# swyoon/Diffusion-by-MaxEntIRL

Hardware: AMD Instinct MI355X
Metric: images/sec (CIFAR-10 DDPM T=10 generation) (higher is better)
Workload: dtype bf16; 1 GPU; CIFAR-10 DDPM U-Net (35.7M params) VARSampler T=10 generation, 256 images/GPU/step, 3x32x32 (BASELINE configs[1]); noise drawn inside the step; global_batch=256, T=10, parallelism=dp1 (independent trajectories, no collective)

## Files before the change

### diffusion-by-maxentirl_amd/csrc/conv_igemm.hip

```cpp
#include "conv_common.h"

namespace {

template <int MB, int NB, int CK, int PMAX>
__global__ __launch_bounds__(256) void conv_igemm_kernel(ConvArgs p) {
    constexpr int WAVES_PX = 8 / NB;
    constexpr int WAVES_CO = 4 / WAVES_PX;
    constexpr int BN = 32 * MB * WAVES_CO;
    constexpr int ROWB = CK * 2 + 16;
    constexpr int KSTEPS = CK / 16;
    constexpr int PPP = CK / 8;
    extern __shared__ __attribute__((aligned(16))) char smem[];

    const int tid = threadIdx.x;
    const int lane = tid & 63;
    const int wave = __builtin_amdgcn_readfirstlane(tid >> 6);
    const int wco = wave % WAVES_CO;
    const int wpx = wave / WAVES_CO;

    int pt, cot;
    if (!conv_block_to_tile(p, blockIdx.x, pt, cot)) return;

    const bool k27 = p.in_mode == DXMI_IN_NCHW_F32_K27;
    const bool rows = p.in_mode == DXMI_IN_ROWS_F32;
// ... 383 lines not shown
    const int HP = flat ? 256 : a.SUBS * a.HH * a.HWd;
    p->lds = (size_t)HP * (CK * 2 + 16);
    b.lds_buf = (int)p->lds;
    const int npieces = HP * (CK / 8);
    const int pmax = npieces <= 6 * 256 ? 6 : (npieces <= 9 * 256 ? 9 : 0);
    const bool wide = a.Cout % 128 == 0 && a.out_mode != DXMI_OUT_NCHW_F32;
    b.CT = wide ? a.Cout / 128 : a.CB;
    p->kind = ConvKernel::igemm;
    p->t0 = wide && variant == 1 ? 2 : 1;
    p->t1 = !wide ? 2 : (variant == 1 ? 4 : 8);
    p->t2 = pmax;
    p->grid = (a.PT + 7) / 8 * 8 * b.CT;
    p->id = p->t0 * 1000 + p->t1 * 100 + pmax;
}

template <int MB, int NB>
int launch_igemm(const ConvPlan& p, hipStream_t st) {
    return p.t2 == 6 ? launch_conv<MB, NB, 32, 6>(p.args, p.lds, st)
                     : p.t2 == 9 ? launch_conv<MB, NB, 32, 9>(p.args, p.lds, st) : launch_conv<MB, NB, 32, 0>(p.args, p.lds, st);
}

void conv_select(const ConvArgs& a, int variant, ConvPlan* p) {
    auto is = [&](bool (*select)(const ConvArgs&, ConvPlan*)) { *p = ConvPlan{}; p->args = a; return select(a, p); };
    if (variant == 0 && (a.gn_out ? is(conv_sm_select) || is(conv_ws8_select)
                                  : is(conv_ws_select) || is(conv1x1_rw8_select) || is(conv1x1_rw_select) || is(conv_head_select) ||
                                        is(conv_sm_select) || is(conv_ws8_select) || is(conv_stem_select) || is(conv_pipe_select)))
        return;
    *p = ConvPlan{};
    p->args = a;
    conv_igemm_select(a, variant, p);
}

int conv_launch(const ConvPlan& p, hipStream_t st) {
    switch (p.kind) {
    case ConvKernel::ws: return conv_ws_launch(p, st);
    case ConvKernel::ws8: return conv_ws8_launch(p, st);
    case ConvKernel::sm: return conv_sm_launch(p, st);
    case ConvKernel::rw: return conv1x1_rw_launch(p, st);
    case ConvKernel::rw8: return conv1x1_rw8_launch(p, st);
    case ConvKernel::head: return conv_head_launch(p, st);
    case ConvKernel::stem: return conv_stem_launch(p, st);
    case ConvKernel::pipe:
    case ConvKernel::stream1x1: return conv_pipe_launch(p, st);
    case ConvKernel::igemm: break;
    }
    if (p.t0 == 2) return launch_igemm<2, 4>(p, st);
    return p.t1 == 8 ? launch_igemm<1, 8>(p, st) : launch_igemm<1, 2>(p, st);
// ... 205 lines not shown
```

### diffusion-by-maxentirl_amd/csrc/conv_ws.hip

```cpp
#include "conv_common.h"
#include <stdlib.h>
#include <type_traits>


#ifdef DXMI_CONV_STAMPS
__device__ unsigned g_ws_wait[256][176];
extern "C" int dxmi_debug_read_ws_stamps(void* dst, int bytes) {
    return (int)hipMemcpyFromSymbol(dst, HIP_SYMBOL(g_ws_wait), bytes, 0, hipMemcpyDeviceToHost);
}
#define WS_STAMPED_BARRIER(idx)                                                                     \
    do {                                                                                            \
        const unsigned long long t0_ = __builtin_amdgcn_s_memtime();                                \
        ws_barrier();                                                                               \
        const unsigned long long t1_ = __builtin_amdgcn_s_memtime();                                \
        if (wave == 0 && lane == 0 && (idx) < 160 && blockIdx.x < 256) g_ws_wait[blockIdx.x][(idx)] = (unsigned)(t1_ - t0_); \
    } while (0)
#define WS_CLOCKSTAMP(slot, cond)                                                                    \
    do {                                                                                            \
        if ((cond) && lane == 0 && blockIdx.x < 256) {                                              \
            g_ws_wait[blockIdx.x][(slot)] = (unsigned)__builtin_amdgcn_s_memtime();                 \
            g_ws_wait[blockIdx.x][(slot) + 1] = (unsigned)__builtin_amdgcn_s_memrealtime();         \
        }                                                                                           \
    } while (0)
#define WS_TSTAMP(slot, cond)                                                                        \
// ... 3 lines not shown
#define WS_DBG(bit) (p.stagger & (bit))
#else
#define WS_STAMPED_BARRIER(idx) ws_barrier()
#define WS_TSTAMP(slot, cond) do {} while (0)
#define WS_CLOCKSTAMP(slot, cond) do {} while (0)
#define WS_DBG(bit) 0
#endif

__device__ unsigned long long g_ws_clock[4];
extern "C" int dxmi_conv_ws_last_clock(unsigned long long* host_out4) {
    return hipMemcpyFromSymbol(host_out4, HIP_SYMBOL(g_ws_clock), 4 * sizeof(unsigned long long), 0, hipMemcpyDeviceToHost) == hipSuccess ? DXMI_OK
                                                                                                                                          : DXMI_ELAUNCH;
}

namespace {

constexpr int WS_A_SLOT = 8192;
constexpr int WS_RING = 6;
constexpr int WS_A_RING = WS_RING * WS_A_SLOT;
constexpr int WS_RO = 256 * 256;
constexpr int WS_TB = 1024;
constexpr int WS_HALO_BLOCKS = 22;
constexpr int WS_HALO = WS_HALO_BLOCKS * 1024;

__device__ uint4 ws_zero16 = {0u, 0u, 0u, 0u};

#define WS_GPTR(p) ((const __attribute__((address_space(1))) void*)(p))
#define WS_LPTR(p) ((__attribute__((address_space(3))) void*)(p))

__device__ __forceinline__ void ws_barrier() { asm volatile("s_waitcnt lgkmcnt(0)\n\ts_barrier" ::: "memory"); }

#define WS_INTERLEAVE_4()                                       \
    do {                                                        \
        _Pragma("unroll") for (int i_ = 0; i_ < 4; ++i_) {      \
            __builtin_amdgcn_sched_group_barrier(0x008, 3, 0);  \
            __builtin_amdgcn_sched_group_barrier(0x100, 1, 0);  \
        }                                                       \
        __builtin_amdgcn_sched_group_barrier(0x008, 4, 0);      \
    } while (0)
#define WS_INTERLEAVE_8()                                       \
    do {                                                        \
        _Pragma("unroll") for (int i_ = 0; i_ < 8; ++i_) {      \
            __builtin_amdgcn_sched_group_barrier(0x008, 1, 0);  \
            __builtin_amdgcn_sched_group_barrier(0x100, 1, 0);  \
        }                                                       \
        __builtin_amdgcn_sched_group_barrier(0x008, 8, 0);      \
// ... 43 lines not shown
                ws_f32x2 x = {__builtin_bit_cast(float, raw[i] << 16), __builtin_bit_cast(float, raw[i] & 0xffff0000u)};
                ws_f32x2 y = x * A[i] + B[i];
                const ws_f32x2 t = y * ws_f32x2{-1.4426950408889634f, -1.4426950408889634f};
                ws_f32x2 e = {__builtin_amdgcn_exp2f(t[0]), __builtin_amdgcn_exp2f(t[1])};
                e = e + ws_f32x2{1.f, 1.f};
                const ws_f32x2 rc = {__builtin_amdgcn_rcpf(e[0]), __builtin_amdgcn_rcpf(e[1])};
                y = y * rc;
                bf16x2 o = {(bf16)y[0], (bf16)y[1]};
                sink ^= __builtin_bit_cast(unsigned, o);
            }
            raw += u32x4{0x10001u, 0x20003u, 0x10002u, 0x30001u};
        }
    }
};
#define WS_VALU_DECL(lane_) WsValuLoad vl_; vl_.init(lane_)
#define WS_VALU_RUN() vl_.run()
#define WS_VALU_DONE() do { if (vl_.sink == 0x12345u) reinterpret_cast<volatile unsigned*>(p.out)[0] = vl_.sink; } while (0)
#else
#define WS_VALU_DECL(lane_) do {} while (0)
#define WS_VALU_RUN() do {} while (0)
#define WS_VALU_DONE() do {} while (0)
#endif

template <int TW>
__device__ __forceinline__ void conv_ws_body(const ConvArgs& p) {
    constexpr int TH = 256 / TW, HP = TW == 32 ? 34 : 18, HH = TH + 2, TWl = TW == 32 ? 5 : 4;
    extern __shared__ __attribute__((aligned(1024))) char smem[];
    char* const halo0 = smem;
    char* const aring = smem + 2 * WS_HALO;
    char* const ro = aring + WS_A_RING;
    float* const tb = reinterpret_cast<float*>(ro + WS_RO);

    const int tid = threadIdx.x, lane = tid & 63;
    const int wave = __builtin_amdgcn_readfirstlane(tid >> 6);
    const int txn = p.OW / TW, tyn = p.OH / TH;
    const int nchunks = (p.C0 + p.C1) / 32;
    const int S = 9 * nchunks;
    const int ntiles = p.PT * p.CT;
    const int ups = p.ups ? 1 : 0;

    auto tile_of = [&](int q, WsTile& t) {
        t.cot = q % p.CT;
        const int pt = q / p.CT;
        const int tx = pt % txn, ty = (pt / txn) % tyn;
        t.n0 = pt / (txn * tyn);
        t.oy0 = ty * TH;
        t.ox0 = tx * TW;
    };

    const int q0 = dxmi_xcd_logical(blockIdx.x, gridDim.x, p.xcd_order);
    int q = q0;
    if (q >= ntiles) return;
    const int qstride = gridDim.x;
    if (blockIdx.x == 0 && tid == 0) {
// ... 51 lines not shown
        (void)stamp_i;
        for (;;) {
            const bool more = q + qstride < ntiles;
            for (int c = 0; c < nchunks; c += 2) {
#pragma unroll
                for (int u = 0; u < 18; ++u) {
                    read_b(u, 1, By);
                    if (u & 1) mfma16(A1, Bx, 0); else mfma16(A0, Bx, 0);
                    WS_INTERLEAVE_4();
                    if (u % 3 == 2) { if (!(WS_DBG(16))) WS_STAMPED_BARRIER(stamp_i + c * 9 + u); }
                    if (u & 1) read_a(u + 1, A0); else read_a(u + 1, A1);
                    read_b(u + 1, 0, Bx);
                    if (u & 1) mfma16(A1, By, 1); else mfma16(A0, By, 1);
                    WS_INTERLEAVE_8();
                    __builtin_amdgcn_sched_barrier(0);
                }
            }
            WS_TSTAMP(158, wave == 0 && q == q0);
            ws_barrier();
            WS_TSTAMP(159, wave == 0 && q == q0);
            {
                const bool plain = p.act == DXMI_ACT_NONE;
                char* const rowb = ro + ((ph * 128 + px) << 8) + 8 * (kg & 1);
                const bool want_stats = p.gn_stats != nullptr;
                const int cot_ = q % p.CT;
                float* const stp = want_stats ? p.gn_stats + ((size_t)((q / p.CT) * 2 + ph) * (p.Cout >> 1) + cot_ * 64 + ch * 32 + kg * 2) * 2 : nullptr;
                auto epi = [&](auto RES, auto MASK, auto ACT, auto STATS) {
                    constexpr bool kRes = decltype(RES)::value, kMask = decltype(MASK)::value, kAct = decltype(ACT)::value, kStats = decltype(STATS)::value;
#pragma unroll
                    for (int cb = 0; cb < 4; ++cb) {
                        float st[4] = {0.f, 0.f, 0.f, 0.f};
                        const int co = ch * 64 + cb * 16 + 4 * kg;
                        const f32x4 b0 = *reinterpret_cast<const f32x4*>(tb + co), t0 = *reinterpret_cast<const f32x4*>(tb + 128 + co);
                        f32x4 bv;
#pragma unroll
                        for (int e = 0; e < 4; ++e) bv[e] = b0[e] + t0[e];
                        char* const a0 = rowb + (((ch * 8 + cb * 2 + (kg >> 1)) ^ px) << 4);
                        bf16x4 r[8];
                        if constexpr (kRes) {
#pragma unroll
                            for (int nb = 0; nb < 8; ++nb) r[nb] = *reinterpret_cast<const bf16x4*>(a0 + nb * 4096);
                        }
#pragma unroll
                        for (int nb = 0; nb < 8; ++nb) {
                            f32x4 v;
#pragma unroll
                            for (int e = 0; e < 4; ++e) v[e] = acc[cb][nb][e] + bv[e];
                            if constexpr (kRes) {
                                if constexpr (kMask) {
#pragma unroll
                                    for (int e = 0; e < 4; ++e) v[e] *= ((float)r[nb][e] > 0.f ? 1.f : p.mask_slope);
                                } else {
#pragma unroll
                                    for (int e = 0; e < 4; ++e) v[e] += (float)r[nb][e];
                                }
                            }
                            if constexpr (kAct) {
#pragma unroll
                                for (int e = 0; e < 4; ++e) v[e] = dxmi_act_lin(v[e], slope);
                            }
                            bf16x4 o;
#pragma unroll
                            for (int e = 0; e < 4; ++e) o[e] = (bf16)v[e];
                            *reinterpret_cast<bf16x4*>(a0 + nb * 4096) = o;
                            if constexpr (kStats) dxmi_stats4(o, st);
#pragma unroll
                            for (int e = 0; e < 4; ++e) acc[cb][nb][e] = 0.f;
                        }
                        if constexpr (kStats) {
#pragma unroll
                            for (int e = 0; e < 4; ++e) st[e] = dxmi_row16_sum(st[e]);
                            if (px == 0 && cot_ * 128 + co < p.Cout) {
                                f32x4 sv;
#pragma unroll
                                for (int e = 0; e < 4; ++e) sv[e] = st[e];
                                *reinterpret_cast<f32x4*>(stp + cb * 16) = sv;
                            }
                        }
                    }
                };
                using T_ = std::true_type;
                using F_ = std::false_type;
                const bool is_mask = has_res && p.res_is_mask;
                if (plain && !is_mask) {
                    if (has_res) { if (want_stats) epi(T_{}, F_{}, F_{}, T_{}); else epi(T_{}, F_{}, F_{}, F_{}); }
                    else { if (want_stats) epi(F_{}, F_{}, F_{}, T_{}); else epi(F_{}, F_{}, F_{}, F_{}); }
                } else if (!want_stats) {
                    if (is_mask) { if (plain) epi(T_{}, T_{}, F_{}, F_{}); else epi(T_{}, T_{}, T_{}, F_{}); }
                    else if (has_res) epi(T_{}, F_{}, T_{}, F_{});
                    else epi(F_{}, F_{}, T_{}, F_{});
                } else {
                    if (is_mask) epi(T_{}, T_{}, T_{}, T_{});
                    else if (has_res) epi(T_{}, F_{}, T_{}, T_{});
                    else epi(F_{}, F_{}, T_{}, T_{});
                }
            }
            WS_TSTAMP(166, wave == 0 && q == q0);
            ws_barrier();
            WS_TSTAMP(157, wave == 0 && q == q0);
            if (!more) {
                WS_CLOCKSTAMP(170, wave == 0);
                break;
            }
            q += qstride;
            stamp_i += S;
        }
    } else if (wave < 6) {
        WS_VALU_DECL(lane);
        const int lw = wave - 4;
        const char* const wb = reinterpret_cast<const char*>(p.w) + (size_t)lane * 16;
        WsTile cur;
        tile_of(q, cur);
        auto issue_tap = [&](int cot, int g) {
            if (WS_DBG(1)) return;
            const int c = g / 9, t = g - c * 9;
            char* dst = aring + (g % WS_RING) * WS_A_SLOT + lw * 4096;
            const char* src = wb + ((size_t)(t * p.KST + c * 2 + lw) * p.CB) * 1024;
#pragma unroll
            for (int f = 0; f < 4; ++f) {
                const int cb = cot * 4 + f < p.CB ? cot * 4 + f : p.CB - 1;
// ... 35 lines not shown
        bool first_tile_l = true, first_group0 = true;
        load_group(0, cur.cot, cur.cot, fq[0]);
        load_group(1, cur.cot, cur.cot, fq[1]);
        asm volatile("s_waitcnt vmcnt(12)" ::: "memory");
        store_group(0, fq[0]);
        asm volatile("s_waitcnt lgkmcnt(0)" ::: "memory");
        load_group(2, cur.cot, cur.cot, fq[0]);
        ws_barrier();
        bool first_tile = true;
        for (;;) {
            const bool more = q + qstride < ntiles;
            WsTile nxt = cur;
            if (more) tile_of(q + qstride, nxt);
            if (!first_tile && lw == 0 && !(WS_DBG(8))) {
                const int co_a = cur.cot * 128 + lane, co_b = co_a + 64 < p.Cout ? co_a + 64 : p.Cout - 1;
                if (p.bias) {
                    __builtin_amdgcn_global_load_lds(WS_GPTR(p.bias + co_a), WS_LPTR(tb), 4, 0, 0);
                    __builtin_amdgcn_global_load_lds(WS_GPTR(p.bias + co_b), WS_LPTR(tb + 64), 4, 0, 0);
                }
                if (p.addvec) {
                    const float* av = p.addvec + (size_t)cur.n0 * p.addvec_ld;
                    __builtin_amdgcn_global_load_lds(WS_GPTR(av + co_a), WS_LPTR(tb + 128), 4, 0, 0);
                    __builtin_amdgcn_global_load_lds(WS_GPTR(av + co_b), WS_LPTR(tb + 192), 4, 0, 0);
                }
            }
            const bf16* const res_t = p.residual + ((((size_t)cur.n0 * p.OH + cur.oy0) * p.OW + cur.ox0) * p.Cout + cur.cot * 128);
            const bool res_here = !first_tile_l && p.residual != nullptr && !(WS_DBG(8));
            first_tile_l = false;
            first_tile = false;
            for (int G0 = 0; G0 < NG; G0 += 2) {
#pragma unroll
                for (int j = 0; j < 2; ++j) {
                    const int G = G0 + j;
                    if (G > 0 || first_group0) {
                        asm volatile("s_waitcnt vmcnt(12)" ::: "memory");
                        store_group(G + 1, fq[(j + 1) & 1]);
                        asm volatile("s_waitcnt lgkmcnt(0)" ::: "memory");
                    }
                    if (res_here && G > 0) {
                        const int cg = (G - 1) / 3, g3 = (G - 1) - cg * 3;
                        if (cg + 1 < nchunks) {
                            const int k0 = cg * kpc_l < 32 ? cg * kpc_l : 32, k1 = k0 + kpc_l < 32 ? k0 + kpc_l : 32;
                            const int i0 = g3 < 2 ? 3 * g3 : 6, i1 = g3 < 2 ? 3 * g3 + 3 : 12;
                            const int ka = k0 + i0 < k1 ? k0 + i0 : k1, kb = k0 + i1 < k1 ? k0 + i1 : k1;
#pragma unroll 1
                            for (int k = ka; k < kb; ++k) {
                                const int rel = ((k >> (TWl - 3)) * p.OW + (k & (TW / 8 - 1)) * 8) * p.Cout + ((k & 1) ? lpar_l1 : lpar_l0);
                                const bool ok = cur.cot * 128 + ((k & 1) ? c8o_l : c8e_l) * 8 < p.Cout;
                                const void* g = ok ? (const void*)(res_t + rel) : (const void*)zero_page_l;
                                __builtin_amdgcn_global_load_lds(WS_GPTR(g), WS_LPTR(ro + (k * 128 + lw * 64) * 16), 16, 0, 0);
                            }
                        }
                    }
                    if (G > 0 || first_group0) load_group(G + 3, cur.cot, more ? nxt.cot : cur.cot, fq[(j + 1) & 1]);
                    WS_TSTAMP(151, wave == 4 && G == 0 && q == q0 + qstride);
                    WS_VALU_RUN();
                    if (!(WS_DBG(16))) ws_barrier();
                }
            }
            first_group0 = false;
            if (more) {
                asm volatile("s_waitcnt vmcnt(12)" ::: "memory");
                store_group(1, fq[1]);
                asm volatile("s_waitcnt lgkmcnt(0)" ::: "memory");
                load_group(3, nxt.cot, nxt.cot, fq[1]);
            }
            ws_barrier();
            ws_barrier();
            WS_TSTAMP(150, wave == 4 && q == q0);
            if (!more) break;
            q += qstride;
            cur = nxt;
        }
        asm volatile("s_waitcnt vmcnt(0)" ::: "memory");
        WS_VALU_DONE();
    } else if (wave == 6) {
        WS_VALU_DECL(lane);
        constexpr int HBA = WS_HALO_BLOCKS;
        const char* const zero_page = reinterpret_cast<const char*>(p.mask_src);
        int hrel0[HBA], hrel1[HBA];
        unsigned m_in = 0, m_top = 0, m_bot = 0, m_left = 0, m_right = 0;
#pragma unroll
        for (int k = 0; k < HBA; ++k) {
            const int hp = k * 16 + (lane >> 2);
            const int hy = hp / HP, hx = hp - hy * HP;
            const int rel = ((hy - 1) >> ups) * p.IW + ((hx - 1) >> ups);
            const int j8 = ((lane & 3) ^ (2 * ((hx >> 2) & 1))) * 8;
            hrel0[k] = (rel * p.C0 + j8) * 2;
            hrel1[k] = (rel * p.C1 + j8) * 2;
            m_in |= (unsigned)(hy < HH && hx < TW + 2) << k;
// ... 23 lines not shown
            for (int k = 0; k < HBA; ++k) {
                if (k < ka || k >= kb) continue;
                const char* g = (hmask >> k) & 1 ? base + (first ? hrel0[k] : hrel1[k]) : zero_page;
                __builtin_amdgcn_global_load_lds(WS_GPTR(g), WS_LPTR(buf + k * 1024), 16, 0, 0);
            }
        };
        WsTile cur;
        tile_of(q, cur);
        if (!p.bias) { tb[lane] = 0.f; tb[64 + lane] = 0.f; }
        if (!p.addvec) { tb[128 + lane] = 0.f; tb[192 + lane] = 0.f; }
        halo_plan(cur);
        halo_issue(0, halo0, 0, HBA);
        if (!(WS_DBG(8))) {
            const int co_a = cur.cot * 128 + lane, co_b = co_a + 64 < p.Cout ? co_a + 64 : p.Cout - 1;
            if (p.bias) {
                __builtin_amdgcn_global_load_lds(WS_GPTR(p.bias + co_a), WS_LPTR(tb), 4, 0, 0);
                __builtin_amdgcn_global_load_lds(WS_GPTR(p.bias + co_b), WS_LPTR(tb + 64), 4, 0, 0);
            }
            if (p.addvec) {
                const float* av = p.addvec + (size_t)cur.n0 * p.addvec_ld;
                __builtin_amdgcn_global_load_lds(WS_GPTR(av + co_a), WS_LPTR(tb + 128), 4, 0, 0);
                __builtin_amdgcn_global_load_lds(WS_GPTR(av + co_b), WS_LPTR(tb + 192), 4, 0, 0);
            }
        }
        asm volatile("s_waitcnt vmcnt(0)" ::: "memory");
        ws_barrier();
        WsTile nxt = cur;
        for (;;) {
            const bool more = q + qstride < ntiles;
            for (int c = 0; c < nchunks; ++c) {
                const bool wrap = c + 1 == nchunks;
                if (wrap && more) {
                    tile_of(q + qstride, nxt);
                    halo_plan(nxt);
                }
                const bool do_halo = !wrap || more;
                char* const hbuf = halo0 + ((c + 1) & 1) * WS_HALO;
                const int hc = wrap ? 0 : c + 1;
#pragma unroll
                for (int t = 0; t < 9; ++t) {
                    if (t < 8 && do_halo) halo_issue(hc, hbuf, 3 * t, 3 * t + 3 < HBA ? 3 * t + 3 : HBA);
                    if (t == 8) asm volatile("s_waitcnt vmcnt(0)" ::: "memory");
                    if (t % 3 == 2) { WS_VALU_RUN(); if (!(WS_DBG(16))) ws_barrier(); }
                }
            }
            ws_barrier();
            ws_barrier();
            if (!more) break;
            q += qstride;
            cur = nxt;
        }
        WS_VALU_DONE();
    } else if (wave == 7) {
        WS_VALU_DECL(lane);
        const char* const zero_page = reinterpret_cast<const char*>(p.mask_src);
        const int prA = lane >> 4, prB = 4 + (lane >> 4), lc = lane & 15;
        const int lparA[2] = {prA * p.Cout + ((lc ^ prA) * 8), prA * p.Cout + ((lc ^ (prA | 8)) * 8)};
        const int lparB[2] = {prB * p.Cout + ((lc ^ prB) * 8), prB * p.Cout + ((lc ^ (prB | 8)) * 8)};
        const int c8A[2] = {lc ^ prA, lc ^ (prA | 8)}, c8B[2] = {lc ^ prB, lc ^ (prB | 8)};
        auto tile_base = [&](const WsTile& t) -> size_t {
            return (((size_t)t.n0 * p.OH + t.oy0) * p.OW + t.ox0) * p.Cout + t.cot * 128;
        };
        auto piece_u = [&](int k) -> int { return ((k >> (TWl - 3)) * p.OW + (k & (TW / 8 - 1)) * 8) * p.Cout; };
        WsTile cur;
        tile_of(q, cur);
        if (p.residual != nullptr && !(WS_DBG(8))) {
            const bf16* rb = p.residual + tile_base(cur);
#pragma unroll 1
            for (int k = 0; k < 32; ++k) {
// ... 29 lines not shown
                    piece_range(c, t, ka, kb);
                    if (ka < kb && do_drain) {
                        bf16x8 va[2], vb[2];
#pragma unroll
                        for (int u = 0; u < 2; ++u)
                            if (ka + u < kb) {
                                va[u] = *reinterpret_cast<const bf16x8*>(ro + ((ka + u) * 128 + lane) * 16);
                                vb[u] = *reinterpret_cast<const bf16x8*>(ro + ((ka + u) * 128 + 64 + lane) * 16);
                            }
#pragma unroll
                        for (int u = 0; u < 2; ++u)
                            if (ka + u < kb) {
                                const int k = ka + u, pu = piece_u(k);
                                if (prev.cot * 128 + c8A[k & 1] * 8 < p.Cout) *reinterpret_cast<bf16x8*>(out_prev + pu + lparA[k & 1]) = va[u];
                                if (prev.cot * 128 + c8B[k & 1] * 8 < p.Cout) *reinterpret_cast<bf16x8*>(out_prev + pu + lparB[k & 1]) = vb[u];
                            }
                    }
                    asm volatile("s_waitcnt lgkmcnt(0)" ::: "memory");
                    if (t % 3 == 2) { WS_VALU_RUN(); if (!(WS_DBG(16))) ws_barrier(); }
                }
            }
            if (!have_prev) asm volatile("s_waitcnt vmcnt(0)" ::: "memory");
            ws_barrier();
            ws_barrier();
            out_prev = reinterpret_cast<bf16*>(p.out) + tile_base(cur);
            prev = cur;
            have_prev = true;
            if (!more) break;
            q += qstride;
            cur = nxt;
        }
        WS_VALU_DONE();
    }

    {
        const int qlast = q0 + ((ntiles - 1 - q0) / qstride) * qstride;
        WsTile lt;
        tile_of(qlast, lt);
        bf16* const ob = reinterpret_cast<bf16*>(p.out) + ((((size_t)lt.n0 * p.OH + lt.oy0) * p.OW + lt.ox0) * p.Cout + lt.cot * 128);
        const int t2 = tid & 127, kq = tid >> 7;
        const int pr = t2 >> 4;
#pragma unroll
        for (int i = 0; i < 8; i += 4) {
            bf16x8 v[4];
#pragma unroll
            for (int u = 0; u < 4; ++u) v[u] = *reinterpret_cast<const bf16x8*>(ro + (((i + u) * 4 + kq) * 128 + t2) * 16);
#pragma unroll
            for (int u = 0; u < 4; ++u) {
                const int k = (i + u) * 4 + kq;
                const int lp = k * 8 + pr;
                const int c8 = (t2 & 15) ^ (lp & 15);
                const int rel = ((lp >> TWl) * p.OW + (lp & (TW - 1))) * p.Cout + c8 * 8;
                if (lt.cot * 128 + c8 * 8 < p.Cout) *reinterpret_cast<bf16x8*>(ob + rel) = v[u];
            }
        }
        WS_CLOCKSTAMP(174, wave == 0);
    }
    if (blockIdx.x == 0 && tid == 0) {
        g_ws_clock[2] = __builtin_amdgcn_s_memtime();
        g_ws_clock[3] = __builtin_amdgcn_s_memrealtime();
    }
}

template <int TW>
__global__ __launch_bounds__(512, 1) void conv_ws_kernel(ConvArgs p) {
    conv_ws_body<TW>(p);
}

}

bool conv_ws_select(const ConvArgs& a, ConvPlan* p) {
    if (a.in_mode != DXMI_IN_NHWC_BF16 || a.out_mode != DXMI_OUT_NHWC_BF16) return false;
    if (a.ksize != 3 || a.stride != 1 || a.pad != 1 || a.ups == 2 || (a.mask_src && a.residual) || a.act == DXMI_ACT_SILU) return false;
    if (a.Cout % 64 != 0 || (a.C0 + a.C1) % 32 != 0 || a.C0 % 32 != 0) return false;
    const int TW = a.OW >= 32 ? 32 : a.OW;
    if (TW != 32 && TW != 16) return false;
    const int TH = 256 / TW;
    if (a.OH % TH != 0 || a.OW % TW != 0) return false;
    const int nchunks = (a.C0 + a.C1) / 32;
    if ((9 * nchunks) % WS_RING != 0 || nchunks % 2 != 0) return false;
    if (nchunks < 4) return false;
    const int min_tiles = dxmi_tuning("conv_ws_min_tiles");
    if ((long)a.N * (a.OH / TH) * (a.OW / TW) * ((a.Cout + 127) / 128) < min_tiles) return false;
    if ((long)a.N * a.IH * a.IW * (a.C0 > a.C1 ? a.C0 : a.C1) * 2 >= (1L << 31)) return false;
    ConvArgs& b = p->args;
    if (a.mask_src) { b.residual = a.mask_src; b.res_is_mask = 1; }
    b.SUBS = 1;
    b.PT = a.N * (a.OH / TH) * (a.OW / TW);
    b.CT = (a.Cout + 127) / 128;
    b.tile_px = 256;
    b.xcd_order = 1;
    b.stagger = 0;
    p->kind = ConvKernel::ws; p->t0 = TW;
    p->grid = b.PT * b.CT < 256 ? b.PT * b.CT : 256;
    p->lds = 2 * WS_HALO + WS_A_RING + WS_RO + WS_TB;
    p->id = 400000 + TW;
    p->stats_tile = 128;
    conv_ws_up_select(a, p);
    return true;
}

int conv_ws_launch(const ConvPlan& p, hipStream_t st) {
    if (p.t1 == 1) return conv_ws_up_launch(p, st);
    static const void* zero_page = nullptr;
    DXMI_CHECK_ARG(conv_zero_page(zero_page, HIP_SYMBOL(ws_zero16)), "dxmi_conv2d_fwd(ws): hipGetSymbolAddress(ws_zero16) failed");
    ConvArgs b = p.args;
    b.mask_src = reinterpret_cast<const bf16*>(zero_page);
#ifdef DXMI_CONV_STAMPS
    static const int dbg = getenv("DXMI_CONV_WS_DBG") ? atoi(getenv("DXMI_CONV_WS_DBG")) : 0;
    b.stagger = dbg;
#endif
    static bool attr_set = false;
    if (!attr_set) {
        (void)hipFuncSetAttribute(reinterpret_cast<const void*>(conv_ws_kernel<32>), hipFuncAttributeMaxDynamicSharedMemorySize, 160 * 1024);
        (void)hipFuncSetAttribute(reinterpret_cast<const void*>(conv_ws_kernel<16>), hipFuncAttributeMaxDynamicSharedMemorySize, 160 * 1024);
        attr_set = true;
    }
    if (p.t0 == 32) hipLaunchKernelGGL(conv_ws_kernel<32>, dim3(p.grid), dim3(512), p.lds, st, b);
    else hipLaunchKernelGGL(conv_ws_kernel<16>, dim3(p.grid), dim3(512), p.lds, st, b);
    DXMI_CHECK_LAUNCH("dxmi_conv2d_fwd(ws)");
    return DXMI_OK;
}
```

### diffusion-by-maxentirl_amd/dxmi_hip/ops.py

```python
import ctypes
import math
import os

import torch

from . import _lib
from . import graph as _graph
from ._lib import ConvDesc, check, load

ACT_NONE, ACT_LEAKY02, ACT_RELU, ACT_SILU = 0, 1, 2, 3
IN_NHWC_BF16, IN_NCHW_F32_K27 = 0, 1
OUT_NHWC_BF16, OUT_NCHW_F32 = 0, 1


_RAW_STREAM = getattr(torch._C, "_cuda_getCurrentRawStream", None)
_GET_DEVICE = getattr(torch._C, "_cuda_getDevice", None)


def _stream():
    if _RAW_STREAM is not None and _GET_DEVICE is not None:
        return ctypes.c_void_p(_RAW_STREAM(_GET_DEVICE()))
    return ctypes.c_void_p(torch.cuda.current_stream().cuda_stream)


# ... 156 lines not shown

def pack_conv_weight(w, transpose_flip=False, k27=False, out=None):
    _need_cuda(w)
    if w.dim() == 2:
        w = w[:, :, None, None]
    w = w.detach().contiguous().float()
    O, I, k, _ = w.shape
    Cout, Cin = (I, O) if transpose_flip else (O, I)
    lib = load()
    nbytes = lib.dxmi_packed_conv_weight_bytes(Cout, Cin, k, int(k27))
    if out is None:
        out = pack_tensor(nbytes, torch.uint8, w.device)
    assert out.numel() == nbytes
    if _PACK_BATCH is not None:
        _PACK_BATCH.append((w, out, Cout, Cin, k, transpose_flip, k27))
    else:
        check(lib.dxmi_pack_conv_weight(_ptr(w), _ptr(out), Cout, Cin, k, int(transpose_flip), int(k27), _stream()),
              "dxmi_pack_conv_weight")
    return PackedConvWeight(out, Cout, Cin, k, k27, transpose_flip)


class BlockStats:

    __slots__ = ("buf", "P")

    def __init__(self, buf, P):
        self.buf, self.P = buf, P


_STATS_P = {}


def conv2d(x, pw, *, in1=None, bias=None, addvec=None, residual=None, stride=1, pad=None, pad_br=None, upsample=False,
           act=ACT_NONE, out=None, out_nchw_f32=False, variant=0, mask_src=None, mask_slope=0.0, want_stats=False, fuse_gn=None):
    _need_cuda(x, in1, bias, addvec, residual, out)
    k = pw.ksize
    if pad is None:
        pad = k // 2
    d = ConvDesc()
    if pw.k27:
        N, _, IH, IW = x.shape
        C0, C1 = 3, 0
        assert x.dtype == torch.float32 and x.is_contiguous()
    else:
        N, IH, IW, C0 = x.shape
        C1 = in1.shape[3] if in1 is not None else 0
        assert x.dtype == torch.bfloat16 and x.is_contiguous()
        assert in1 is None or (in1.dtype == torch.bfloat16 and in1.is_contiguous() and in1.shape[:3] == x.shape[:3])
        assert C0 + C1 == pw.Cin, f"conv2d: input channels {C0}+{C1} != packed Cin {pw.Cin}"
    VIH, VIW = (IH * 2, IW * 2) if upsample else (IH, IW)
    if pad_br is None:
        pad_br = pad
    OH, OW = (VIH + pad + pad_br - k) // stride + 1, (VIW + pad + pad_br - k) // stride + 1
    Cout = pw.Cout
    if out is None:
        if out_nchw_f32:
            out = torch.empty((N, Cout, OH, OW), dtype=torch.float32, device=x.device)
# ... 11 lines not shown
        assert residual.dtype == torch.bfloat16 and residual.is_contiguous() and tuple(residual.shape) == (N, OH, OW, Cout)
    d.residual = residual.data_ptr() if residual is not None else None
    d.out = out.data_ptr()
    d.N, d.IH, d.IW, d.C0, d.C1, d.OH, d.OW, d.Cout = N, IH, IW, C0, C1, OH, OW, Cout
    d.ksize, d.stride, d.pad, d.upsample, d.act = k, stride, pad, int(upsample), act
    d.in_mode = IN_NCHW_F32_K27 if pw.k27 else IN_NHWC_BF16
    d.out_mode = OUT_NCHW_F32 if out_nchw_f32 else OUT_NHWC_BF16
    d.variant = variant
    if mask_src is not None:
        assert mask_src.dtype == torch.bfloat16 and mask_src.is_contiguous() and tuple(mask_src.shape) == (N, OH, OW, Cout)
    d.mask_src = mask_src.data_ptr() if mask_src is not None else None
    d.mask_slope = float(mask_slope)
    d.gn_stats = None
    stats = None
    if want_stats and not out_nchw_f32 and variant == 0:
        key = (N, IH, IW, C0, C1, OH, OW, Cout, k, stride, pad, int(upsample), act, d.in_mode, residual is not None, mask_src is not None)
        P = _STATS_P.get(key)
        if P is None:
            P = _STATS_P[key] = int(load().dxmi_conv2d_gn_stats_partials(ctypes.byref(d)))
        if P > 0:
            stats = BlockStats(torch.empty((N, P, Cout // 2, 2), dtype=torch.float32, device=x.device), P)
            d.gn_stats = stats.buf.data_ptr()
    d.gn_out, y = None, None
    if fuse_gn is not None:
        assert not want_stats
        gamma, beta, groups, eps, silu, keep_raw = fuse_gn
        d.gn_groups = groups
        d.gn_flags = int(bool(silu)) | (0 if keep_raw else 2)
        key = ("gn", N, IH, IW, C0, C1, OH, OW, Cout, k, stride, pad, int(upsample), act, d.in_mode, d.out_mode, variant,
               residual is not None, mask_src is not None, groups, bool(keep_raw))
        ok = _STATS_P.get(key)
        if ok is None:
            ok = _STATS_P[key] = int(load().dxmi_conv2d_gn_fuse_supported(ctypes.byref(d)))
        if ok:
            assert gamma.dtype == torch.float32 and beta.dtype == torch.float32 and gamma.numel() == Cout and beta.numel() == Cout
            y = torch.empty((N, OH, OW, Cout), dtype=torch.bfloat16, device=x.device)
            d.gn_out, d.gn_gamma, d.gn_beta, d.gn_eps = y.data_ptr(), gamma.data_ptr(), beta.data_ptr(), float(eps)
    if PROFILER is not None:
        PROFILER.launch_conv(d)
    else:
        check(load().dxmi_conv2d_fwd(ctypes.byref(d), _stream()), "dxmi_conv2d_fwd")
    if fuse_gn is not None:
        return (out if (y is None or fuse_gn[5]) else None), y
    if stats is not None and stats.P > MAX_APPLY_PARTIALS:
        stats = fold_stats(stats)
    return (out, stats) if want_stats else out


class OpProfiler:

    def __init__(self):
        self.records = []

    def bracket(self, cls, name, flops, nbytes, fn):
        e0, e1 = torch.cuda.Event(enable_timing=True), torch.cuda.Event(enable_timing=True)
        e0.record()
        out = fn()
        e1.record()
        self.records.append((cls, name, float(flops), float(nbytes), e0, e1))
        return out

    def launch_conv(self, d):
        lib = load()
        kid = lib.dxmi_conv2d_kernel_id(ctypes.byref(d))
        cin = 27 if d.in_mode == IN_NCHW_F32_K27 else (d.C0 + d.C1) * d.ksize * d.ksize
        flops = 2.0 * d.N * d.OH * d.OW * d.Cout * cin
        in_b = d.N * d.IH * d.IW * (d.C0 + d.C1) * (4 if d.in_mode == IN_NCHW_F32_K27 else 2)
        out_b = d.N * d.OH * d.OW * d.Cout * (4 if d.out_mode == OUT_NCHW_F32 else 2)
        res_b = out_b if d.residual else 0
        if d.gn_out:
            res_b += out_b if not (d.gn_flags & 2) else 0
        w_b = d.Cout * cin * 2
        cls = "conv_other" if kid >= 600000 else "conv1x1" if kid >= 500000 else "conv3x3" if kid >= 400000 else "conv_stem" if kid >= 300000 else ("conv1x1" if kid >= 200000 else ("conv3x3" if kid >= 30000 else "conv_other"))
        if kid == 400008 and d.gn_out:
            kid = 400009
        self.bracket(cls, kid, flops, in_b + out_b + res_b + w_b,
                     lambda: check(lib.dxmi_conv2d_fwd(ctypes.byref(d), _stream()), "dxmi_conv2d_fwd"))

    def summary(self):
        out = {}
        for cls, name, fl, by, e0, e1 in self.records:
            s = out.setdefault((cls, name), {"launches": 0, "ms": 0.0, "flops": 0.0, "bytes": 0.0})
            s["launches"] += 1
            s["ms"] += e0.elapsed_time(e1)
            s["flops"] += fl
            s["bytes"] += by
        return out


PROFILER = None


def _prof(cls, name, flops, nbytes, fn):
    return fn() if PROFILER is None else PROFILER.bracket(cls, name, flops, nbytes, fn)


_WS = {}

# ... 1804 lines not shown
```

### diffusion-by-maxentirl_amd/models/DxMI/unet_small.py

```python
import os

import torch
import torch.nn as nn

from dxmi_hip import ops
from dxmi_hip._lib import DxmiError
from dxmi_hip.packs import PackedWeights, WeightPacks


def Normalize(in_channels):
    return nn.GroupNorm(num_groups=32, num_channels=in_channels, eps=1e-6, affine=True)


def _conv(cin, cout, k, stride=1, padding=0):
    return nn.Conv2d(cin, cout, kernel_size=k, stride=stride, padding=padding)


class Upsample(nn.Module):

    def __init__(self, in_channels, with_conv):
        super().__init__()
        self.with_conv = with_conv
        if with_conv:
            self.conv = _conv(in_channels, in_channels, 3, 1, 1)
# ... 142 lines not shown
            ps.pack((id(b), "conv2"), b.conv2.weight)
            if b.in_channels != b.out_channels:
                sc = b.conv_shortcut if b.use_conv_shortcut else b.nin_shortcut
                ps.pack((id(b), "short"), sc.weight)
        for m in self.modules():
            if isinstance(m, AttnBlock):
                ps.pack((id(m), "qkv"), ps.stage_cat([m.q.weight, m.k.weight, m.v.weight]))
                pk[id(m), "qkv_bias"] = ps.stage_cat([m.q.bias, m.k.bias, m.v.bias])
                ps.pack((id(m), "proj"), m.proj_out.weight)
                if m.in_channels == 256:
                    ps.derived((id(m), "proj_attn"), lambda out, m=m: ops.pack_attn_proj_weight(m.proj_out.weight, out=out))
                    ps.derived((id(m), "block"), lambda out, m=m: ops.attn_block_pack(
                        m.q.weight, m.q.bias, m.k.weight, m.v.weight, m.v.bias, m.proj_out.weight, m.proj_out.bias,
                        float(int(m.in_channels) ** (-0.5)), out=out))
            elif isinstance(m, (Upsample, Downsample)):
                ps.pack((id(m), "conv"), m.conv.weight)
        ps.pack("conv_in", self.conv_in.weight, k27=(self.in_channels == 3))
        ps.pack("conv_out", self.conv_out.weight)

    FUSE_ATTN_PROJ = True
    FUSE_GN_SHORTCUT = os.environ.get("DXMI_GN_SHORTCUT", "1") != "0"
    FUSE_ATTN_BLOCK = True
    FUSE_GN_SMALL = True
    STREAM_GN_MIN_HW = 256

    def _conv_s(self, x, pw, **kw):
        out, st = ops.conv2d(x, pw, want_stats=True, **kw)
        if st is None and out.shape[1] * out.shape[2] >= self.STREAM_GN_MIN_HW:
            st = ops.block_stats(out)
        return out, st

    def _resblock(self, pk, b, x0, x1, tp, s0=None, s1=None, nxt=None):
        stream = x0.shape[1] * x0.shape[2] >= self.STREAM_GN_MIN_HW
        fused = None
        if isinstance(s0, _Normed):
            assert s0.norm is b.norm1 and x1 is None
            a0 = s0.y
        else:
            if self.FUSE_GN_SHORTCUT and stream and b.in_channels != b.out_channels and not b.use_conv_shortcut:
                fused = ops.groupnorm_silu_shortcut(x0, b.norm1.weight, b.norm1.bias, pk[id(b), "short"], in1=x1, bias=b.nin_shortcut.bias,
                                                    eps=1e-6, silu=True, stats=(s0, s1))
            if fused is not None:
                a0, sc = fused
            else:
                a0 = ops.groupnorm_silu(x0, b.norm1.weight, b.norm1.bias, in1=x1, eps=1e-6, silu=True, stats=(s0, s1))
        off = pk[id(b), "toff"]
        a = None
        if not stream and self.FUSE_GN_SMALL:
            h, a = ops.conv2d(a0, pk[id(b), "conv1"], bias=b.conv1.bias, addvec=tp[:, off:off + b.out_channels],
                              fuse_gn=(b.norm2.weight, b.norm2.bias, 32, 1e-6, True, False))
            sh = None
            if a is None and stream:
                sh = ops.block_stats(h)
        else:
            h, sh = ops.conv2d(a0, pk[id(b), "conv1"], bias=b.conv1.bias, addvec=tp[:, off:off + b.out_channels], want_stats=True)
        if a is None:
            a = ops.groupnorm_silu(h, b.norm2.weight, b.norm2.bias, eps=1e-6, silu=True, stats=(sh, None))
        if b.in_channels != b.out_channels:
            if fused is None:
                sc_mod = b.conv_shortcut if b.use_conv_shortcut else b.nin_shortcut
                sc = ops.conv2d(x0, pk[id(b), "short"], in1=x1, bias=sc_mod.bias)
        else:
            assert x1 is None
            sc = x0
        if stream:
            return self._conv_s(a, pk[id(b), "conv2"], bias=b.conv2.bias, residual=sc)
        if nxt is not None and self.FUSE_GN_SMALL:
            h, y = ops.conv2d(a, pk[id(b), "conv2"], bias=b.conv2.bias, residual=sc,
                              fuse_gn=(nxt[0].weight, nxt[0].bias, 32, 1e-6, nxt[1], True))
            return h, (None if y is None else _Normed(y, nxt[0]))
        return ops.conv2d(a, pk[id(b), "conv2"], bias=b.conv2.bias, residual=sc), None

    def _attn(self, pk, m, x, sx=None):
        N, H, W, C = x.shape
        if self.FUSE_ATTN_BLOCK and (id(m), "block") in pk and isinstance(sx, ops.BlockStats) and ops.attn_block_supported(H * W, C, 1):
            return ops.attn_block(x, sx, m.norm.weight, m.norm.bias, pk[id(m), "block"], eps=1e-6, want_stats=True)
# ... 98 lines not shown
```

Baseline: 7120 images/s.

## Fuse GroupNorm+SiLU epilogue into warp-specialized conv for 16x16 resblock conv1

Adds a GN variant of the warp-specialized 3x3 conv kernel. When a tile covers a whole 16x16 image, the kernel reduces per-group statistics in LDS, then normalizes and applies SiLU to the output tile in place before it is written. The resblock conv1 on streaming-resolution layers requests this path through a new norm_next argument, which removes the separate groupnorm_silu pass and its extra read and write of the activation. The cost is extra barriers and LDS per tile, and the raw conv output is no longer stored (keep_raw is false).

```diff
diff --git a/diffusion-by-maxentirl_amd/csrc/conv_igemm.hip b/diffusion-by-maxentirl_amd/csrc/conv_igemm.hip
--- a/diffusion-by-maxentirl_amd/csrc/conv_igemm.hip
+++ b/diffusion-by-maxentirl_amd/csrc/conv_igemm.hip
@@ -429,7 +429,7 @@
 
 void conv_select(const ConvArgs& a, int variant, ConvPlan* p) {
     auto is = [&](bool (*select)(const ConvArgs&, ConvPlan*)) { *p = ConvPlan{}; p->args = a; return select(a, p); };
-    if (variant == 0 && (a.gn_out ? is(conv_sm_select) || is(conv_ws8_select)
+    if (variant == 0 && (a.gn_out ? ((a.gn_flags & 4) && is(conv_ws_select)) || is(conv_sm_select) || is(conv_ws8_select)
                                   : is(conv_ws_select) || is(conv1x1_rw8_select) || is(conv1x1_rw_select) || is(conv_head_select) ||
                                         is(conv_sm_select) || is(conv_ws8_select) || is(conv_stem_select) || is(conv_pipe_select)))
         return;
diff --git a/diffusion-by-maxentirl_amd/csrc/conv_ws.hip b/diffusion-by-maxentirl_amd/csrc/conv_ws.hip
--- a/diffusion-by-maxentirl_amd/csrc/conv_ws.hip
+++ b/diffusion-by-maxentirl_amd/csrc/conv_ws.hip
@@ -1,4 +1,5 @@
 #include "conv_common.h"
+#include "gn_common.h"
 #include <stdlib.h>
 #include <type_traits>
 
@@ -49,6 +50,7 @@
 constexpr int WS_TB = 1024;
 constexpr int WS_HALO_BLOCKS = 22;
 constexpr int WS_HALO = WS_HALO_BLOCKS * 1024;
+constexpr int WS_GN = 2048;
 
 __device__ uint4 ws_zero16 = {0u, 0u, 0u, 0u};
 
@@ -138,7 +140,7 @@
 #define WS_VALU_DONE() do {} while (0)
 #endif
 
-template <int TW>
+template <int TW, bool GN>
 __device__ __forceinline__ void conv_ws_body(const ConvArgs& p) {
     constexpr int TH = 256 / TW, HP = TW == 32 ? 34 : 18, HH = TH + 2, TWl = TW == 32 ? 5 : 4;
     extern __shared__ __attribute__((aligned(1024))) char smem[];
@@ -146,6 +148,8 @@
     char* const aring = smem + 2 * WS_HALO;
     char* const ro = aring + WS_A_RING;
     float* const tb = reinterpret_cast<float*>(ro + WS_RO);
+    float* const gb = tb + WS_TB / 4;
+    float* const ps = gb + 256;
 
     const int tid = threadIdx.x, lane = tid & 63;
     const int wave = __builtin_amdgcn_readfirstlane(tid >> 6);
@@ -243,9 +247,9 @@
             {
                 const bool plain = p.act == DXMI_ACT_NONE;
                 char* const rowb = ro + ((ph * 128 + px) << 8) + 8 * (kg & 1);
-                const bool want_stats = p.gn_stats != nullptr;
+                const bool want_stats = GN || p.gn_stats != nullptr;
                 const int cot_ = q % p.CT;
-                float* const stp = want_stats ? p.gn_stats + ((size_t)((q / p.CT) * 2 + ph) * (p.Cout >> 1) + cot_ * 64 + ch * 32 + kg * 2) * 2 : nullptr;
+                float* const stp = p.gn_stats ? p.gn_stats + ((size_t)((q / p.CT) * 2 + ph) * (p.Cout >> 1) + cot_ * 64 + ch * 32 + kg * 2) * 2 : nullptr;
                 auto epi = [&](auto RES, auto MASK, auto ACT, auto STATS) {
                     constexpr bool kRes = decltype(RES)::value, kMask = decltype(MASK)::value, kAct = decltype(ACT)::value, kStats = decltype(STATS)::value;
 #pragma unroll
@@ -285,8 +289,10 @@
                             for (int e = 0; e < 4; ++e) o[e] = (bf16)v[e];
                             *reinterpret_cast<bf16x4*>(a0 + nb * 4096) = o;
                             if constexpr (kStats) dxmi_stats4(o, st);
-#pragma unroll
-                            for (int e = 0; e < 4; ++e) acc[cb][nb][e] = 0.f;
+                            if constexpr (!GN) {
+#pragma unroll
+                                for (int e = 0; e < 4; ++e) acc[cb][nb][e] = 0.f;
+                            }
                         }
                         if constexpr (kStats) {
 #pragma unroll
@@ -295,7 +301,8 @@
                                 f32x4 sv;
 #pragma unroll
                                 for (int e = 0; e < 4; ++e) sv[e] = st[e];
-                                *reinterpret_cast<f32x4*>(stp + cb * 16) = sv;
+                                if (!GN || stp) *reinterpret_cast<f32x4*>(stp + cb * 16) = sv;
+                                if constexpr (GN) *reinterpret_cast<f32x4*>(ps + ph * 128 + co) = sv;
                             }
                         }
                     }
@@ -317,6 +324,50 @@
                 }
             }
             WS_TSTAMP(166, wave == 0 && q == q0);
+            if constexpr (GN) {
+                ws_barrier();
+                const int c8 = lane & 15;
+                const f32x4 h0a = *reinterpret_cast<const f32x4*>(ps + c8 * 8), h0b = *reinterpret_cast<const f32x4*>(ps + c8 * 8 + 4);
+                const f32x4 h1a = *reinterpret_cast<const f32x4*>(ps + 128 + c8 * 8), h1b = *reinterpret_cast<const f32x4*>(ps + 128 + c8 * 8 + 4);
+                const f32x4 g0 = *reinterpret_cast<const f32x4*>(gb + c8 * 8), g1 = *reinterpret_cast<const f32x4*>(gb + c8 * 8 + 4);
+                const f32x4 b0 = *reinterpret_cast<const f32x4*>(gb + 128 + c8 * 8), b1 = *reinterpret_cast<const f32x4*>(gb + 128 + c8 * 8 + 4);
+                float2 pair_r[4];
+#pragma unroll
+                for (int k = 0; k < 4; ++k) {
+                    const float s0 = k < 2 ? h0a[2 * k] : h0b[2 * k - 4], q0_ = k < 2 ? h0a[2 * k + 1] : h0b[2 * k - 3];
+                    const float s1 = k < 2 ? h1a[2 * k] : h1b[2 * k - 4], q1_ = k < 2 ? h1a[2 * k + 1] : h1b[2 * k - 3];
+                    float s = 0.f, qq = 0.f;
+                    s += s0;
+                    qq += q0_;
+                    s += s1;
+                    qq += q1_;
+                    pair_r[k] = make_float2(s, qq);
+                }
+                float mean, rstd;
+                gn_group_moments(pair_r, 0, 8, p.OH * p.OW, p.gn_eps, &mean, &rstd);
+                float A[8], Bv[8];
+#pragma unroll
+                for (int e = 0; e < 8; ++e) gn_channel_ab(mean, rstd, e < 4 ? g0[e] : g1[e - 4], e < 4 ? b0[e] : b1[e - 4], A[e], Bv[e]);
+                char* const trow = ro + ((wave * 64 + (lane >> 4)) << 8);
+                auto transform = [&](auto SILU) {
+#pragma unroll
+                    for (int j = 0; j < 16; j += 4) {
+                        bf16x8 v[4];
+#pragma unroll
+                        for (int u = 0; u < 4; ++u) v[u] = *reinterpret_cast<const bf16x8*>(trow + (j + u) * 1024 + ((c8 ^ ((lane >> 4) + 4 * u)) << 4));
+#pragma unroll
+                        for (int u = 0; u < 4; ++u)
+                            *reinterpret_cast<bf16x8*>(trow + (j + u) * 1024 + ((c8 ^ ((lane >> 4) + 4 * u)) << 4)) = gn_norm8(v[u], A, Bv, decltype(SILU)::value);
+                    }
+                };
+                if (p.gn_flags & 1) transform(std::true_type{}); else transform(std::false_type{});
+#pragma unroll
+                for (int cb = 0; cb < 4; ++cb)
+#pragma unroll
+                    for (int nb = 0; nb < 8; ++nb)
+#pragma unroll
+                        for (int e = 0; e < 4; ++e) acc[cb][nb][e] = 0.f;
+            }
             ws_barrier();
             WS_TSTAMP(157, wave == 0 && q == q0);
             if (!more) {
@@ -398,6 +449,12 @@
                     const float* av = p.addvec + (size_t)cur.n0 * p.addvec_ld;
                     __builtin_amdgcn_global_load_lds(WS_GPTR(av + co_a), WS_LPTR(tb + 128), 4, 0, 0);
                     __builtin_amdgcn_global_load_lds(WS_GPTR(av + co_b), WS_LPTR(tb + 192), 4, 0, 0);
+                }
+                if constexpr (GN) {
+                    __builtin_amdgcn_global_load_lds(WS_GPTR(p.gn_gamma + co_a), WS_LPTR(gb), 4, 0, 0);
+                    __builtin_amdgcn_global_load_lds(WS_GPTR(p.gn_gamma + co_b), WS_LPTR(gb + 64), 4, 0, 0);
+                    __builtin_amdgcn_global_load_lds(WS_GPTR(p.gn_beta + co_a), WS_LPTR(gb + 128), 4, 0, 0);
+                    __builtin_amdgcn_global_load_lds(WS_GPTR(p.gn_beta + co_b), WS_LPTR(gb + 192), 4, 0, 0);
                 }
             }
             const bf16* const res_t = p.residual + ((((size_t)cur.n0 * p.OH + cur.oy0) * p.OW + cur.ox0) * p.Cout + cur.cot * 128);
@@ -442,6 +499,7 @@
                 load_group(3, nxt.cot, nxt.cot, fq[1]);
             }
             ws_barrier();
+            if constexpr (GN) ws_barrier();
             ws_barrier();
             WS_TSTAMP(150, wave == 4 && q == q0);
             if (!more) break;
@@ -511,6 +569,12 @@
                 __builtin_amdgcn_global_load_lds(WS_GPTR(av + co_a), WS_LPTR(tb + 128), 4, 0, 0);
                 __builtin_amdgcn_global_load_lds(WS_GPTR(av + co_b), WS_LPTR(tb + 192), 4, 0, 0);
             }
+            if constexpr (GN) {
+                __builtin_amdgcn_global_load_lds(WS_GPTR(p.gn_gamma + co_a), WS_LPTR(gb), 4, 0, 0);
+                __builtin_amdgcn_global_load_lds(WS_GPTR(p.gn_gamma + co_b), WS_LPTR(gb + 64), 4, 0, 0);
+                __builtin_amdgcn_global_load_lds(WS_GPTR(p.gn_beta + co_a), WS_LPTR(gb + 128), 4, 0, 0);
+                __builtin_amdgcn_global_load_lds(WS_GPTR(p.gn_beta + co_b), WS_LPTR(gb + 192), 4, 0, 0);
+            }
         }
         asm volatile("s_waitcnt vmcnt(0)" ::: "memory");
         ws_barrier();
@@ -534,6 +598,7 @@
                 }
             }
             ws_barrier();
+            if constexpr (GN) ws_barrier();
             ws_barrier();
             if (!more) break;
             q += qstride;
@@ -609,6 +674,7 @@
             }
             if (!have_prev) asm volatile("s_waitcnt vmcnt(0)" ::: "memory");
             ws_barrier();
+            if constexpr (GN) ws_barrier();
             ws_barrier();
             out_prev = reinterpret_cast<bf16*>(p.out) + tile_base(cur);
             prev = cur;
@@ -651,7 +717,12 @@
 
 template <int TW>
 __global__ __launch_bounds__(512, 1) void conv_ws_kernel(ConvArgs p) {
-    conv_ws_body<TW>(p);
+    conv_ws_body<TW, false>(p);
+}
+
+template <int TW>
+__global__ __launch_bounds__(512, 1) void conv_ws_gn_kernel(ConvArgs p) {
+    conv_ws_body<TW, true>(p);
 }
 
 }
@@ -670,8 +741,11 @@
     const int min_tiles = dxmi_tuning("conv_ws_min_tiles");
     if ((long)a.N * (a.OH / TH) * (a.OW / TW) * ((a.Cout + 127) / 128) < min_tiles) return false;
     if ((long)a.N * a.IH * a.IW * (a.C0 > a.C1 ? a.C0 : a.C1) * 2 >= (1L << 31)) return false;
+    const bool gn_ok = (a.gn_flags & 4) && (a.gn_flags & 2) && a.OW == 16 && a.OH == 16 && a.Cout % 128 == 0 && !a.ups && !a.residual && !a.mask_src;
+    if (a.gn_out && !gn_ok) return false;
     ConvArgs& b = p->args;
     if (a.mask_src) { b.residual = a.mask_src; b.res_is_mask = 1; }
+    if (a.gn_out) b.out = a.gn_out;
     b.SUBS = 1;
     b.PT = a.N * (a.OH / TH) * (a.OW / TW);
     b.CT = (a.Cout + 127) / 128;
@@ -683,6 +757,12 @@
     p->lds = 2 * WS_HALO + WS_A_RING + WS_RO + WS_TB;
     p->id = 400000 + TW;
     p->stats_tile = 128;
+    p->gn_out = gn_ok;
+    if (a.gn_out) {
+        p->t2 = 1;
+        p->lds += WS_GN;
+        return true;
+    }
     conv_ws_up_select(a, p);
     return true;
 }
@@ -701,9 +781,11 @@
     if (!attr_set) {
         (void)hipFuncSetAttribute(reinterpret_cast<const void*>(conv_ws_kernel<32>), hipFuncAttributeMaxDynamicSharedMemorySize, 160 * 1024);
         (void)hipFuncSetAttribute(reinterpret_cast<const void*>(conv_ws_kernel<16>), hipFuncAttributeMaxDynamicSharedMemorySize, 160 * 1024);
+        (void)hipFuncSetAttribute(reinterpret_cast<const void*>(conv_ws_gn_kernel<16>), hipFuncAttributeMaxDynamicSharedMemorySize, 160 * 1024);
         attr_set = true;
     }
-    if (p.t0 == 32) hipLaunchKernelGGL(conv_ws_kernel<32>, dim3(p.grid), dim3(512), p.lds, st, b);
+    if (p.t2 == 1) hipLaunchKernelGGL(conv_ws_gn_kernel<16>, dim3(p.grid), dim3(512), p.lds, st, b);
+    else if (p.t0 == 32) hipLaunchKernelGGL(conv_ws_kernel<32>, dim3(p.grid), dim3(512), p.lds, st, b);
     else hipLaunchKernelGGL(conv_ws_kernel<16>, dim3(p.grid), dim3(512), p.lds, st, b);
     DXMI_CHECK_LAUNCH("dxmi_conv2d_fwd(ws)");
     return DXMI_OK;
diff --git a/diffusion-by-maxentirl_amd/dxmi_hip/ops.py b/diffusion-by-maxentirl_amd/dxmi_hip/ops.py
--- a/diffusion-by-maxentirl_amd/dxmi_hip/ops.py
+++ b/diffusion-by-maxentirl_amd/dxmi_hip/ops.py
@@ -202,17 +202,20 @@
 
 class BlockStats:
 
-    __slots__ = ("buf", "P")
+    __slots__ = ("buf", "P", "normed")
 
     def __init__(self, buf, P):
         self.buf, self.P = buf, P
+        self.normed = None
 
 
 _STATS_P = {}
+GN_FLAG_WS = 4
 
 
 def conv2d(x, pw, *, in1=None, bias=None, addvec=None, residual=None, stride=1, pad=None, pad_br=None, upsample=False,
-           act=ACT_NONE, out=None, out_nchw_f32=False, variant=0, mask_src=None, mask_slope=0.0, want_stats=False, fuse_gn=None):
+           act=ACT_NONE, out=None, out_nchw_f32=False, variant=0, mask_src=None, mask_slope=0.0, want_stats=False, fuse_gn=None,
+           gn_ws=False, norm_next=None):
     _need_cuda(x, in1, bias, addvec, residual, out)
     k = pw.ksize
     if pad is None:
@@ -270,16 +273,24 @@
             stats = BlockStats(torch.empty((N, P, Cout // 2, 2), dtype=torch.float32, device=x.device), P)
             d.gn_stats = stats.buf.data_ptr()
     d.gn_out, y = None, None
-    if fuse_gn is not None:
-        assert not want_stats
-        gamma, beta, groups, eps, silu, keep_raw = fuse_gn
+    assert norm_next is None or (fuse_gn is None and want_stats)
+    fuse = fuse_gn if norm_next is None else (tuple(norm_next) + (False,) if stats is not None else None)
+    if fuse is not None:
+        assert not want_stats or norm_next is not None
+        gamma, beta, groups, eps, silu, keep_raw = fuse
+        ws_too = bool(gn_ws) or norm_next is not None
         d.gn_groups = groups
-        d.gn_flags = int(bool(silu)) | (0 if keep_raw else 2)
+        d.gn_flags = int(bool(silu)) | (0 if keep_raw else 2) | (GN_FLAG_WS if ws_too else 0)
         key = ("gn", N, IH, IW, C0, C1, OH, OW, Cout, k, stride, pad, int(upsample), act, d.in_mode, d.out_mode, variant,
-               residual is not None, mask_src is not None, groups, bool(keep_raw))
+               residual is not None, mask_src is not None, groups, bool(keep_raw), ws_too, norm_next is not None)
         ok = _STATS_P.get(key)
         if ok is None:
-            ok = _STATS_P[key] = int(load().dxmi_conv2d_gn_fuse_supported(ctypes.byref(d)))
+            ok = int(load().dxmi_conv2d_gn_fuse_supported(ctypes.byref(d)))
+            if ok and norm_next is not None:
+                d.gn_flags &= ~GN_FLAG_WS
+                ok = int(not load().dxmi_conv2d_gn_fuse_supported(ctypes.byref(d)))
+                d.gn_flags |= GN_FLAG_WS
+            _STATS_P[key] = ok
         if ok:
             assert gamma.dtype == torch.float32 and beta.dtype == torch.float32 and gamma.numel() == Cout and beta.numel() == Cout
             y = torch.empty((N, OH, OW, Cout), dtype=torch.bfloat16, device=x.device)
@@ -288,10 +299,13 @@
         PROFILER.launch_conv(d)
     else:
         check(load().dxmi_conv2d_fwd(ctypes.byref(d), _stream()), "dxmi_conv2d_fwd")
+    if stats is not None and stats.P > MAX_APPLY_PARTIALS:
+        stats = fold_stats(stats)
     if fuse_gn is not None:
         return (out if (y is None or fuse_gn[5]) else None), y
-    if stats is not None and stats.P > MAX_APPLY_PARTIALS:
-        stats = fold_stats(stats)
+    if y is not None:
+        stats.normed = y
+        return None, stats
     return (out, stats) if want_stats else out
 
 
@@ -322,6 +336,8 @@
         cls = "conv_other" if kid >= 600000 else "conv1x1" if kid >= 500000 else "conv3x3" if kid >= 400000 else "conv_stem" if kid >= 300000 else ("conv1x1" if kid >= 200000 else ("conv3x3" if kid >= 30000 else "conv_other"))
         if kid == 400008 and d.gn_out:
             kid = 400009
+        if kid == 400016 and d.gn_out:
+            kid = 400116
         self.bracket(cls, kid, flops, in_b + out_b + res_b + w_b,
                      lambda: check(lib.dxmi_conv2d_fwd(ctypes.byref(d), _stream()), "dxmi_conv2d_fwd"))
 
diff --git a/diffusion-by-maxentirl_amd/models/DxMI/unet_small.py b/diffusion-by-maxentirl_amd/models/DxMI/unet_small.py
--- a/diffusion-by-maxentirl_amd/models/DxMI/unet_small.py
+++ b/diffusion-by-maxentirl_amd/models/DxMI/unet_small.py
@@ -188,6 +188,7 @@
     FUSE_GN_SHORTCUT = os.environ.get("DXMI_GN_SHORTCUT", "1") != "0"
     FUSE_ATTN_BLOCK = True
     FUSE_GN_SMALL = True
+    FUSE_GN_STREAM = os.environ.get("DXMI_GN_STREAM", "1") != "0"
     STREAM_GN_MIN_HW = 256
 
     def _conv_s(self, x, pw, **kw):
@@ -218,6 +219,10 @@
             sh = None
             if a is None and stream:
                 sh = ops.block_stats(h)
+        elif stream and self.FUSE_GN_STREAM:
+            h, sh = ops.conv2d(a0, pk[id(b), "conv1"], bias=b.conv1.bias, addvec=tp[:, off:off + b.out_channels], want_stats=True,
+                               norm_next=(b.norm2.weight, b.norm2.bias, 32, 1e-6, True))
+            a = sh.normed if sh is not None else None
         else:
             h, sh = ops.conv2d(a0, pk[id(b), "conv1"], bias=b.conv1.bias, addvec=tp[:, off:off + b.out_channels], want_stats=True)
         if a is None:
```

Result: faster. 7213 images/s (median of 6 runs) (+1.3%).
